# nanoporetech/dorado

Hardware: NVIDIA H100
Metric: basecalled samples/s (higher is better)
Workload: dtype f16 (fp32 accumulate; fp32 decode)

## Files before the change

dorado_b200/csrc/decode.cu:

```cuda
#include "decode.h"

#include "b200_crf_math.h"
#include "common.cuh"
#include "engine.h"
#include "nvtx.h"

#include <string>

namespace b200 {

namespace {

constexpr int kBeamW = 32;
constexpr uint32_t kCrcPoly = 0x82f63b78u;
constexpr uint32_t kCrcSeed = 0x12345678u;

template <int SL>
struct Dims {
    static constexpr int S = 1 << (2 * SL);
    static constexpr int C = 4 * S;
};

template <int SL>
struct ScanCfg {
    static constexpr int S = Dims<SL>::S, C = Dims<SL>::C, P4 = S / 4;
    static constexpr int SPT = S > 512 ? S / 512 : 1;
    static constexpr int NT = S / SPT;
    static constexpr int PITCH = P4 + 2;
};

__device__ __forceinline__ float clampf(float v, float c) {
    const float ce = c > 0.0f ? c : __int_as_float(0x7f800000);
    return fminf(fmaxf(v, -ce), ce);
}

template <int SL>
__global__ void __launch_bounds__(ScanCfg<SL>::S > 256 ? ScanCfg<SL>::S : 256)
        crf_bwd_scan_kernel(const __half* __restrict__ scores, float* __restrict__ bwd, int N, int T_pitch, float clamp_val,
                            float blank, const int32_t* __restrict__ lens, int stride) {
    using Cfg = ScanCfg<SL>;
    constexpr int S = Cfg::S, C = Cfg::C, P4 = Cfg::P4, PITCH = Cfg::PITCH;
    constexpr int CH = S >= 256 ? 1 : 256 / S;
    constexpr int PF = 4;
    const int g = threadIdx.x / S;
    const int v = threadIdx.x % S;
    const int chunk = blockIdx.x * CH + g;
    __shared__ __align__(16) float a[CH][2][S];
    __shared__ float st[CH][2][16 * PITCH];
    const bool active = chunk < N;
    const int chunk_c = active ? chunk : N - 1;
    const int T = lens ? min(T_pitch, __ldg(lens + chunk_c) / stride) : T_pitch;
    const uint2* srow = reinterpret_cast<const uint2*>(scores + (size_t)chunk_c * T_pitch * C) + v;
    constexpr int RS = C / 4;
    float* out = bwd + (size_t)chunk_c * (T_pitch + 1) * S;
    const int q = v % P4, top = v / P4;
    const int st_row = 4 * (v & 3), st_col = v >> 2;

    uint2 pf[PF];
#pragma unroll
    for (int k = 0; k < PF; ++k) {
        const int tt = T - 1 - k;
        if (tt >= 0) pf[k] = __ldg(srow + (size_t)tt * RS);
    }
    auto stage = [&](int buf, const uint2& r) {
        const __half2 h0 = *reinterpret_cast<const __half2*>(&r.x), h1 = *reinterpret_cast<const __half2*>(&r.y);
        const float2 f0 = __half22float2(h0), f1 = __half22float2(h1);
        float* d = &st[g][buf][st_row * PITCH + st_col];
        d[0] = clampf(f0.x, clamp_val);
        d[PITCH] = clampf(f0.y, clamp_val);
        d[2 * PITCH] = clampf(f1.x, clamp_val);
        d[3 * PITCH] = clampf(f1.y, clamp_val);
    };
    float own = 0.0f;
    a[g][0][v] = 0.0f;
    if (active) out[(size_t)T * S + v] = 0.0f;
    stage(0, pf[0]);
    if (T - 1 - PF >= 0) pf[0] = __ldg(srow + (size_t)(T - 1 - PF) * RS);
    if constexpr (S <= 32) __syncwarp(); else named_bar_sync(1 + g, S);

    int cur = 0;
    for (int t = T - 1; t >= 0; t -= PF) {
#pragma unroll
        for (int k = 0; k < PF; ++k) {
            const int tt = t - k;
            if (tt >= 0) {
                if (tt - 1 >= 0) {
                    stage(cur ^ 1, pf[(k + 1) % PF]);
                    if (tt - 1 - PF >= 0) pf[(k + 1) % PF] = __ldg(srow + (size_t)(tt - 1 - PF) * RS);
// ... 453 lines not shown
                    if (d) d[9] = clock64();
                    float vsum[SPT];
                    float lmax = B200_FLT_LOWEST;
#pragma unroll
                    for (int e = 0; e < SPT; ++e) {
                        const uint2 r = pf[k][e];
                        const float bw = pb[k][e];
                        if (t + PF < T) {
                            pf[k][e] = __ldg(reinterpret_cast<const uint2*>(srow + (size_t)(t + PF) * C) + e);
                            pb[k][e] = __ldg(brow + (size_t)(t + PF + 1) * S + e);
                        }
                        const float2 f0 = __half22float2(*reinterpret_cast<const __half2*>(&r.x));
                        const float2 f1 = __half22float2(*reinterpret_cast<const __half2*>(&r.y));
                        const float s0 = clampf(f0.x, clamp_val), s1 = clampf(f0.y, clamp_val);
                        const float s2 = clampf(f1.x, clamp_val), s3 = clampf(f1.y, clamp_val);
                        const int st = SPT * v + e;
                        {
                            const __half2 c0 = __floats2half2_rn(s0, s1), c1 = __floats2half2_rn(s2, s3);
                            uint2 pk;
                            pk.x = *reinterpret_cast<const uint32_t*>(&c0);
                            pk.y = *reinterpret_cast<const uint32_t*>(&c1);
                            *reinterpret_cast<uint2*>(&sc_row[g][slot][4 * st]) = pk;
                        }
                        bw_row[g][slot][st] = bw;
                        const int p = st >> 2;
                        f[e] = b200_lse5(B200_ADD(f[e], blank), B200_ADD(fa[g][cur][p], s0), B200_ADD(fa[g][cur][p + P4], s1),
                                         B200_ADD(fa[g][cur][p + 2 * P4], s2), B200_ADD(fa[g][cur][p + 3 * P4], s3));
                        fa[g][cur ^ 1][st] = f[e];
                        vsum[e] = B200_ADD(f[e], bw);
                        lmax = b200_fmaxf(lmax, vsum[e]);
                    }
                    float mx = warp_max(lmax);
                    if constexpr (NW > 1) {
                        if (lane == 0) red[g][0][wv] = mx;
                        named_bar_sync(BAR_SCAN, NT);
                        mx = red[g][0][0];
#pragma unroll
                        for (int w = 1; w < NW; ++w) mx = b200_fmaxf(mx, red[g][0][w]);
                    }
                    float ex[SPT];
                    float part = 0.0f;
#pragma unroll
                    for (int e = 0; e < SPT; ++e) {
                        ex[e] = b200_expf_nonpos(B200_SUB(vsum[e], mx));
                        part = e == 0 ? ex[0] : B200_ADD(part, ex[e]);
                    }
#pragma unroll
                    for (int o = 16; o >= 1; o >>= 1) part = B200_ADD(part, __shfl_xor_sync(0xffffffffu, part, o));
                    float z = part;
                    if constexpr (NW > 1) {
                        if (lane == 0) red[g][1][wv] = part;
                        named_bar_sync(BAR_SCAN, NT);
                        z = red[g][1][0];
#pragma unroll
                        for (int w = 1; w < NW; ++w) z = B200_ADD(z, red[g][1][w]);
                    }
#pragma unroll
                    for (int e = 0; e < SPT; ++e) post_row[g][slot][SPT * v + e] = B200_DIV(ex[e], z);
                    named_bar_arrive(BAR_FULL + slot, GT);
                    if (d) d[10] = clock64();
                    cur ^= 1;
                }
            }
        }
    } else {
        named_bar_sync(BAR_SCAN, GT);
        BeamLane me{0u, 0u, 0.0f};
        int width = beam_init<SL>(bw_row[g][1], bsm[g], me, W, lane);
        named_bar_sync(BAR_SCAN, GT);
        for (int t = 0; t < T; ++t) {
            const int slot = t & 1;
            long long* d = (dbg && chunk == 0 && t >= 100 && t < 108) ? dbg + (t - 100) * 16 : nullptr;
            if (d && lane == 0) d[7] = clock64();
            named_bar_sync(BAR_FULL + slot, GT);
            width = beam_step<SL>(sc_row[g][slot], bw_row[g][slot], post_row[g][slot], bsm[g], me, width, W, log_beam_cut, blank,
                                  t == T - 1, meta_out + (size_t)t * kBeamW, prob_out + (size_t)t * kBeamW, lane, d);
            if (t + 2 < T) named_bar_arrive(BAR_EMPTY + slot, GT);
        }
    }
}

constexpr int kWarpDecodeMaxChunks = 16;
constexpr int kWarpStPitch = 16 + 2;

struct WarpDecodeSmem {
    __align__(16) float fa[2][64];
    float st[16 * kWarpStPitch];
    __align__(16) __half sc_row[256];
    __align__(16) float bw_row[64];
    __align__(16) float post_row[64];
    BeamSmem bs;
};

__device__ __forceinline__ float4 clamped_scores(const uint2& r, float clamp_val) {
    const float2 f0 = __half22float2(*reinterpret_cast<const __half2*>(&r.x));
    const float2 f1 = __half22float2(*reinterpret_cast<const __half2*>(&r.y));
    return make_float4(clampf(f0.x, clamp_val), clampf(f0.y, clamp_val), clampf(f1.x, clamp_val), clampf(f1.y, clamp_val));
}

__global__ void __launch_bounds__(kWarpDecodeMaxChunks * 32, 1) crf_decode_warp_kernel(const __half* __restrict__ scores,
                                                                                      float* __restrict__ bwd,
                                                                                      uint2* __restrict__ beam,
                                                                                      int N,
                                                                                      int T_pitch,
                                                                                      float clamp_val,
                                                                                      float blank,
                                                                                      int W,
                                                                                      float log_beam_cut,
                                                                                      const int32_t* __restrict__ lens,
                                                                                      int stride) {
    constexpr int S = Dims<3>::S, C = Dims<3>::C, P4 = S / 4, PITCH = kWarpStPitch;
    constexpr int RS = C / 4;
    constexpr int PF = 4;
    extern __shared__ __align__(16) unsigned char warp_decode_smem[];
    const int w = threadIdx.x >> 5, lane = threadIdx.x & 31;
    const int chunk = blockIdx.x * (blockDim.x >> 5) + w;
    if (chunk >= N) return;
    WarpDecodeSmem& sm = reinterpret_cast<WarpDecodeSmem*>(warp_decode_smem)[w];
    const int T = lens ? min(T_pitch, __ldg(lens + chunk) / stride) : T_pitch;
    const uint2* srow = reinterpret_cast<const uint2*>(scores + (size_t)chunk * T_pitch * C);
    float* brow = bwd + (size_t)chunk * (T_pitch + 1) * S;
    const int s0 = lane, s1 = lane + 32;

    {
        const int q = lane & 15, top = lane >> 4;
        auto stage = [&](const uint2& r, int v) {
            const float4 f = clamped_scores(r, clamp_val);
            float* d = &sm.st[4 * (v & 3) * PITCH + (v >> 2)];
            d[0] = f.x;
            d[PITCH] = f.y;
            d[2 * PITCH] = f.z;
            d[3 * PITCH] = f.w;
        };
        uint2 pf[PF][2];
#pragma unroll
        for (int k = 0; k < PF; ++k) {
            const int tt = T - 1 - k;
            if (tt >= 0) {
                pf[k][0] = __ldg(srow + (size_t)tt * RS + s0);
                pf[k][1] = __ldg(srow + (size_t)tt * RS + s1);
            }
        }
        float own0 = 0.0f, own1 = 0.0f;
        sm.fa[0][s0] = 0.0f;
        sm.fa[0][s1] = 0.0f;
        brow[(size_t)T * S + s0] = 0.0f;
        brow[(size_t)T * S + s1] = 0.0f;
        int cur = 0;
        for (int t = T - 1; t >= 0; t -= PF) {
#pragma unroll
            for (int k = 0; k < PF; ++k) {
                const int tt = t - k;
                if (tt >= 0) {
                    stage(pf[k][0], s0);
                    stage(pf[k][1], s1);
                    if (tt - PF >= 0) {
                        pf[k][0] = __ldg(srow + (size_t)(tt - PF) * RS + s0);
                        pf[k][1] = __ldg(srow + (size_t)(tt - PF) * RS + s1);
                    }
                    __syncwarp();
                    const float4 nx = *reinterpret_cast<const float4*>(&sm.fa[cur][4 * q]);
                    const float* sa = &sm.st[top * PITCH + q];
                    const float* sb = &sm.st[(top + 2) * PITCH + q];
                    own0 = b200_lse5(B200_ADD(own0, blank), B200_ADD(nx.x, sa[0]), B200_ADD(nx.y, sa[4 * PITCH]),
                                     B200_ADD(nx.z, sa[8 * PITCH]), B200_ADD(nx.w, sa[12 * PITCH]));
                    own1 = b200_lse5(B200_ADD(own1, blank), B200_ADD(nx.x, sb[0]), B200_ADD(nx.y, sb[4 * PITCH]),
                                     B200_ADD(nx.z, sb[8 * PITCH]), B200_ADD(nx.w, sb[12 * PITCH]));
                    sm.fa[cur ^ 1][s0] = own0;
                    sm.fa[cur ^ 1][s1] = own1;
                    brow[(size_t)tt * S + s0] = own0;
                    brow[(size_t)tt * S + s1] = own1;
                    __syncwarp();
                    cur ^= 1;
                }
            }
        }
    }
    __syncwarp();

    uint32_t* meta_out = reinterpret_cast<uint32_t*>(beam) + (size_t)chunk * T_pitch * kBeamW;
    float* prob_out = reinterpret_cast<float*>(beam) + ((size_t)N + chunk) * T_pitch * kBeamW;
    sm.fa[0][s0] = 0.0f;
    sm.fa[0][s1] = 0.0f;
    sm.bw_row[s0] = brow[s0];
    sm.bw_row[s1] = brow[s1];
    __syncwarp();
    BeamLane me{0u, 0u, 0.0f};
    int width = beam_init<3>(sm.bw_row, sm.bs, me, W, lane);
    uint2 r0n{}, r1n{};
    float b0n = 0.0f, b1n = 0.0f;
    if (T > 0) {
        r0n = __ldg(srow + s0);
        r1n = __ldg(srow + s1);
        b0n = brow[S + s0];
        b1n = brow[S + s1];
    }
    float f0 = 0.0f, f1 = 0.0f;
    int cur = 0;
    const int p0 = s0 >> 2, p1 = s1 >> 2;
    for (int t = 0; t < T; ++t) {
        const uint2 r0 = r0n, r1 = r1n;
        const float bw0 = b0n, bw1 = b1n;
        if (t + 1 < T) {
            r0n = __ldg(srow + (size_t)(t + 1) * RS + s0);
            r1n = __ldg(srow + (size_t)(t + 1) * RS + s1);
            b0n = brow[(size_t)(t + 2) * S + s0];
            b1n = brow[(size_t)(t + 2) * S + s1];
        }
        const float4 c0 = clamped_scores(r0, clamp_val), c1 = clamped_scores(r1, clamp_val);
        {
            const __half2 h00 = __floats2half2_rn(c0.x, c0.y), h01 = __floats2half2_rn(c0.z, c0.w);
            const __half2 h10 = __floats2half2_rn(c1.x, c1.y), h11 = __floats2half2_rn(c1.z, c1.w);
            *reinterpret_cast<uint2*>(&sm.sc_row[4 * s0]) =
                    make_uint2(*reinterpret_cast<const uint32_t*>(&h00), *reinterpret_cast<const uint32_t*>(&h01));
            *reinterpret_cast<uint2*>(&sm.sc_row[4 * s1]) =
                    make_uint2(*reinterpret_cast<const uint32_t*>(&h10), *reinterpret_cast<const uint32_t*>(&h11));
        }
        sm.bw_row[s0] = bw0;
        sm.bw_row[s1] = bw1;
        const float* fc = sm.fa[cur];
        f0 = b200_lse5(B200_ADD(f0, blank), B200_ADD(fc[p0], c0.x), B200_ADD(fc[p0 + P4], c0.y), B200_ADD(fc[p0 + 2 * P4], c0.z),
                       B200_ADD(fc[p0 + 3 * P4], c0.w));
        f1 = b200_lse5(B200_ADD(f1, blank), B200_ADD(fc[p1], c1.x), B200_ADD(fc[p1 + P4], c1.y), B200_ADD(fc[p1 + 2 * P4], c1.z),
                       B200_ADD(fc[p1 + 3 * P4], c1.w));
        sm.fa[cur ^ 1][s0] = f0;
        sm.fa[cur ^ 1][s1] = f1;
        const float v0 = B200_ADD(f0, bw0), v1 = B200_ADD(f1, bw1);
        const float mx = warp_max(b200_fmaxf(v0, v1));
        const float e0 = b200_expf_nonpos(B200_SUB(v0, mx)), e1 = b200_expf_nonpos(B200_SUB(v1, mx));
        float z0 = e0, z1 = e1;
#pragma unroll
        for (int o = 16; o >= 1; o >>= 1) {
            z0 = B200_ADD(z0, __shfl_xor_sync(0xffffffffu, z0, o));
            z1 = B200_ADD(z1, __shfl_xor_sync(0xffffffffu, z1, o));
        }
        const float z = B200_ADD(z0, z1);
        sm.post_row[s0] = B200_DIV(e0, z);
        sm.post_row[s1] = B200_DIV(e1, z);
        __syncwarp();
        width = beam_step<3>(sm.sc_row, sm.bw_row, sm.post_row, sm.bs, me, width, W, log_beam_cut, blank, t == T - 1,
                             meta_out + (size_t)t * kBeamW, prob_out + (size_t)t * kBeamW, lane, nullptr);
        cur ^= 1;
    }
}

int warp_decode_chunks_per_cta(int N, int runners) {
    const int R = runners > 1 ? runners : 1;
    const int per = (int)(((long long)N * R + kNumSMs - 1) / kNumSMs);
    return per < 1 ? 1 : (per > kWarpDecodeMaxChunks ? kWarpDecodeMaxChunks : per);
}

constexpr int kTbTile = 32;
constexpr int kTbWarps = 2;

__host__ __device__ constexpr size_t traceback_warp_bytes(int T) {
    return ((size_t)kTbTile * kBeamW * 4 + (size_t)((T + 3) & ~3) * (4 + 4 + 2) + 16 + 15) & ~(size_t)15;
}

__global__ void __launch_bounds__(kTbWarps * 32) crf_traceback_kernel(const uint32_t* __restrict__ beam_meta,
                                                                      const float* __restrict__ beam_prob,
                                                                      int N,
                                                                      int T_pitch,
                                                                      const int32_t* __restrict__ lens,
                                                                      int stride,
                                                                      const b200_qtable* __restrict__ qtable,
                                                                      uint8_t* __restrict__ moves_out,
                                                                      char* __restrict__ seq_out,
                                                                      char* __restrict__ qstr_out,
                                                                      int32_t* __restrict__ n_bases_out) {
    extern __shared__ __align__(16) unsigned char tb_smem[];
    __shared__ b200_qtable qt;
    for (int i = threadIdx.x; i < (int)(sizeof(b200_qtable) / 4); i += blockDim.x) {
        reinterpret_cast<uint32_t*>(&qt)[i] = reinterpret_cast<const uint32_t*>(qtable)[i];
    }
    __syncthreads();
    const int w = threadIdx.x >> 5, lane = threadIdx.x & 31;
    const int chunk = blockIdx.x * kTbWarps + w;
    if (chunk >= N) return;
    const int T = lens ? min(T_pitch, __ldg(lens + chunk) / stride) : T_pitch;
    const int Tp = (T_pitch + 3) & ~3;
    unsigned char* base = tb_smem + (size_t)w * traceback_warp_bytes(T_pitch);
    uint32_t* tile = reinterpret_cast<uint32_t*>(base);
    uint32_t* path = tile + kTbTile * kBeamW;
    float* pprob = reinterpret_cast<float*>(path + Tp);
    uint16_t* bstart = reinterpret_cast<uint16_t*>(pprob + Tp);

    const uint32_t* mrow = beam_meta + (size_t)chunk * T_pitch * kBeamW + lane;
    uint32_t nxt[kTbTile];
    auto load_tile = [&](int t_hi) {
        const int t_lo = t_hi - kTbTile;
#pragma unroll
        for (int r = 0; r < kTbTile; ++r) {
            const int t = t_lo + r;
            nxt[r] = t >= 0 ? __ldg(mrow + (size_t)t * kBeamW) : 0u;
        }
    };
    if (T > 0) load_tile(T);
    uint32_t ei = 0;
    for (int t_hi = T; t_hi > 0; t_hi -= kTbTile) {
#pragma unroll
        for (int r = 0; r < kTbTile; ++r) tile[r * kBeamW + lane] = nxt[r];
        __syncwarp();
        if (t_hi - kTbTile > 0) load_tile(t_hi - kTbTile);
        if (lane == 0) {
            const int t_lo = t_hi - kTbTile;
            const int r_lo = t_lo < 0 ? -t_lo : 0;
            for (int r = kTbTile - 1; r >= r_lo; --r) {
                const uint32_t e = tile[r * kBeamW + ei];
                path[t_lo + r] = (e & 0xffffu) | ((((e >> 24) & 1u) ^ 1u) << 16) | (ei << 24);
                ei = (e >> 16) & 0xffu;
            }
        }
        __syncwarp();
    }
    if (lane == 0 && T > 0) path[0] |= 1u << 16;
    __syncwarp();
    {
        const float* prow = beam_prob + (size_t)chunk * T_pitch * kBeamW;
        for (int t = lane; t < T; t += 32) {
            pprob[t] = b200_pow0p4f(__ldg(prow + (size_t)t * kBeamW + (path[t] >> 24)));
        }
    }
    __syncwarp();

    int nb = 0;
    for (int t0 = 0; t0 < T; t0 += 32) {
        const int t = t0 + lane;
        const bool m = t < T && ((path[t] >> 16) & 1u);
        const uint32_t bal = __ballot_sync(0xffffffffu, m);
        if (m) bstart[nb + __popc(bal & ((1u << lane) - 1u))] = (uint16_t)t;
        nb += __popc(bal);
    }
    if (lane == 0) bstart[nb] = (uint16_t)T;
    __syncwarp();

    uint8_t* mo = moves_out + (size_t)chunk * T_pitch;
    char* so = seq_out + (size_t)chunk * T_pitch;
    char* qo = qstr_out + (size_t)chunk * T_pitch;
    for (int t = lane; t < T_pitch; t += 32) mo[t] = t < T ? (uint8_t)((path[t] >> 16) & 1u) : 0;
    for (int p = lane; p < T_pitch; p += 32) {
        char sc = 0, qc = 0;
        if (p < nb) {
            const int b0 = bstart[p], b1 = bstart[p + 1];
            float bp = 0.0f, tp = 0.0f;
            int base = 0;
            for (int blk = b0; blk < b1; ++blk) {
                base = path[blk] & 3;
                const float prob = pprob[blk];
                const float wrong = B200_DIV(B200_SUB(1.0f, prob), 3.0f);
                bp = B200_ADD(bp, prob);
#pragma unroll
                for (int k = 0; k < 4; ++k) tp = B200_ADD(tp, k == base ? prob : wrong);
            }
            sc = "ACGT"[path[b0] & 3];
            qc = b200_qtable_lookup(&qt, bp, tp);
        }
        so[p] = sc;
        qo[p] = qc;
    }
    if (lane == 0) n_bases_out[chunk] = nb;
}

size_t traceback_smem_bytes(int T) { return kTbWarps * traceback_warp_bytes(T); }

void launch_traceback(const DecodeArgs& a, cudaStream_t stream, ProfileSink* prof) {
    const size_t smem = traceback_smem_bytes(a.T);
    if (smem > 48 * 1024) ensure_dynamic_smem(crf_traceback_kernel, 200 * 1024);
    const int grid = (a.N + kTbWarps - 1) / kTbWarps;
    NvtxRange r("decode");
    const uint32_t* meta = reinterpret_cast<const uint32_t*>(a.beam);
    const float* prob = reinterpret_cast<const float*>(a.beam) + (size_t)a.N * a.T * kBeamW;
    crf_traceback_kernel<<<grid, kTbWarps * 32, smem, stream>>>(meta, prob, a.N, a.T, a.lens, a.stride, a.qtable, a.moves,
                                                                a.sequence, a.qstring, a.n_bases);
    if (prof) prof->mark("crf_traceback", stream);
}

void launch_decode_warp(const DecodeArgs& a, cudaStream_t stream, ProfileSink* prof) {
    {
        const int cpc = warp_decode_chunks_per_cta(a.N, a.runners);
        const int grid = (a.N + cpc - 1) / cpc;
        const size_t smem = (size_t)cpc * sizeof(WarpDecodeSmem);
        ensure_dynamic_smem(crf_decode_warp_kernel, (int)(kWarpDecodeMaxChunks * sizeof(WarpDecodeSmem)));
        NvtxRange r("beam_search");
        crf_decode_warp_kernel<<<grid, cpc * 32, smem, stream>>>(a.scores, a.bwd, a.beam, a.N, a.T, a.clamp_val, a.blank,
                                                                 a.beam_width, a.log_beam_cut, a.lens, a.stride);
        if (prof) prof->mark("crf_fwd_beam", stream);
    }
    launch_traceback(a, stream, prof);
    B200_CUDA(cudaGetLastError());
}

template <int SL>
void launch_decode(const DecodeArgs& a, cudaStream_t stream, ProfileSink* prof) {
    {
        constexpr int S = Dims<SL>::S;
        constexpr int CH = S >= 256 ? 1 : 256 / S;
        const int grid = (a.N + CH - 1) / CH;
        NvtxRange r("back_guides");
        crf_bwd_scan_kernel<SL><<<grid, S * CH, 0, stream>>>(a.scores, a.bwd, a.N, a.T, a.clamp_val, a.blank, a.lens, a.stride);
        if (prof) prof->mark("crf_bwd_scan", stream);
    }
    {
        using F = FwdCfg<SL>;
        const int grid = (a.N + F::CH - 1) / F::CH;
        NvtxRange r("beam_search");
        crf_fwd_beam_kernel<SL><<<grid, F::THREADS, 0, stream>>>(a.scores, a.bwd, a.beam, a.N, a.T, a.clamp_val, a.blank,
                                                                   a.beam_width, a.log_beam_cut, a.lens, a.stride, a.dbg);
        if (prof) prof->mark("crf_fwd_beam", stream);
    }
    launch_traceback(a, stream, prof);
    B200_CUDA(cudaGetLastError());
}

}

size_t decode_max_blocks() {
    int T = 65535;
    while (traceback_smem_bytes(T) > 200 * 1024) T -= 64;
    return (size_t)T;
}

void carve_decode_scratch(Bump& b, int N, int T, int state_len, float** bwd, uint2** beam) {
    const size_t S = (size_t)1 << (2 * state_len);
    *bwd = b.take<float>((size_t)N * (T + 1) * S * sizeof(float));
    *beam = b.take<uint2>((size_t)N * T * kBeamW * sizeof(uint2));
}

int decode_launches(int state_len) { return state_len == 3 ? 2 : 3; }

void decode_scores(const DecodeArgs& a, cudaStream_t stream, ProfileSink* prof) {
    if (a.beam_width < 1 || a.beam_width > kBeamW) {
        throw std::invalid_argument("b200 decode: beam_width must be in [1, 32]");
    }
    if (a.T < 1 || a.T > 65535 || a.N < 1) {
        throw std::invalid_argument("b200 decode: need 1 <= T <= 65535 and N >= 1");
    }
    if (!a.qtable) throw std::invalid_argument("b200 decode: quality table missing");
    if (a.lens && a.stride < 1) throw std::invalid_argument("b200 decode: chunk lengths need the model stride");
    if (traceback_smem_bytes(a.T) > 200 * 1024) {
        throw std::invalid_argument("b200 decode: " + std::to_string(a.T) + " blocks per chunk exceed what the traceback kernel "
                                    "holds in shared memory (about 10 700); use a smaller chunk size");
    }
    switch (a.state_len) {
        case 3: launch_decode_warp(a, stream, prof); break;
        case 4: launch_decode<4>(a, stream, prof); break;
        case 5: launch_decode<5>(a, stream, prof); break;
        default: throw std::invalid_argument("b200 decode: state_len must be 3, 4 or 5");
    }
}

}
```

dorado_b200/csrc/decode.h:

```cpp
#pragma once

#include <cuda_fp16.h>
#include <cuda_runtime.h>
#include <stddef.h>
#include <stdint.h>
#include "b200_crf_math.h"

namespace b200 {

struct DecodeArgs {
    const __half* scores;
    int N;
    int T;
    int state_len;
    float clamp_val;
    int beam_width;
    float log_beam_cut;
    float blank;
    float q_shift;
    float q_scale;
    const b200_qtable* qtable;
    const int32_t* lens;
    int stride;
    int runners;
    long long* dbg;
    float* bwd;
    uint2* beam;
    uint8_t* moves;
    char* sequence;
    char* qstring;
    int32_t* n_bases;
};

size_t decode_max_blocks();
class Bump;
void carve_decode_scratch(Bump& b, int N, int T, int state_len, float** bwd, uint2** beam);
int decode_launches(int state_len);
struct ProfileSink;
void decode_scores(const DecodeArgs& args, cudaStream_t stream, ProfileSink* prof = nullptr);

}
```

dorado_b200/csrc/engine.cu:

```cuda
#include "engine.h"

#include "b200_crf_math.h"
#include "decode.h"
#include "nvtx.h"

#include <algorithm>
#include <cstdio>
#include <cstdlib>
#include <cmath>
#include <cstring>
#include <limits>
#include <set>
#include <utility>
#include <vector>

namespace b200 {

void ensure_dynamic_smem(const void* kernel, int bytes) {
    static std::mutex mu;
    static std::set<std::pair<int, const void*>> done;
    int dev = 0;
    B200_CUDA(cudaGetDevice(&dev));
    std::lock_guard<std::mutex> lock(mu);
    if (done.count({dev, kernel})) return;
// ... 469 lines not shown
        run_decode(num_chunks);
        B200_CUDA(cudaEventRecord(m_ev[2], s));
        B200_CUDA(cudaStreamSynchronize(s));
        m_plan->check_errors();
        float ms = 0;
        B200_CUDA(cudaEventElapsedTime(&ms, m_ev[0], m_ev[1]));
        fwd += ms;
        B200_CUDA(cudaEventElapsedTime(&ms, m_ev[1], m_ev[2]));
        dec += ms;
    }
    *total_ms = fwd + dec;
    if (forward_ms) *forward_ms = fwd;
    if (decode_ms) *decode_ms = dec;
}

void pipelined_steps(Runner** rs, int R, int num_chunks, int iters, float* total_ms) {
    if (R < 1 || !rs || iters < 1) throw std::invalid_argument("pipelined_steps: bad arguments");
    for (int r = 0; r < R; ++r) {
        if (!rs[r]) throw std::invalid_argument("pipelined_steps: null runner");
        if (&rs[r]->m_engine != &rs[0]->m_engine) throw std::invalid_argument("pipelined_steps: runners of different engines");
        if (num_chunks < 1 || num_chunks > rs[r]->m_N) throw std::invalid_argument("pipelined_steps: num_chunks out of range");
        for (int q = 0; q < r; ++q) {
            if (rs[q] == rs[r]) throw std::invalid_argument("pipelined_steps: the same runner twice");
        }
    }
    std::vector<Runner*> order(rs, rs + R);
    std::sort(order.begin(), order.end());
    std::vector<std::unique_lock<std::mutex>> locks;
    for (Runner* r : order) locks.emplace_back(r->m_mutex);
    Runner& r0 = *rs[0];
    B200_CUDA(cudaSetDevice(r0.m_engine.device()));
    B200_CUDA(cudaEventRecord(r0.m_ev[0], r0.m_stream));
    for (int r = 1; r < R; ++r) B200_CUDA(cudaStreamWaitEvent(rs[r]->m_stream, r0.m_ev[0], 0));
    for (int i = 0; i < iters; ++i) {
        Runner& ru = *rs[i % R];
        ru.run_forward(num_chunks);
        ru.run_decode(num_chunks);
    }
    for (int r = 1; r < R; ++r) {
        B200_CUDA(cudaEventRecord(rs[r]->m_ev[2], rs[r]->m_stream));
        B200_CUDA(cudaStreamWaitEvent(r0.m_stream, rs[r]->m_ev[2], 0));
    }
    B200_CUDA(cudaEventRecord(r0.m_ev[1], r0.m_stream));
    B200_CUDA(cudaStreamSynchronize(r0.m_stream));
    for (int r = 0; r < R; ++r) rs[r]->m_plan->check_errors();
    B200_CUDA(cudaEventElapsedTime(total_ms, r0.m_ev[0], r0.m_ev[1]));
}

void Runner::forward_scores_to_host(int num_chunks, uint16_t* scores_out) {
    if (num_chunks < 1 || num_chunks > m_N) throw std::invalid_argument("forward_scores: num_chunks out of range");
    std::lock_guard<std::mutex> lock(m_mutex);
    B200_CUDA(cudaSetDevice(m_engine.device()));
    cudaStream_t s = m_stream;
    stage_input(num_chunks);
    run_forward(num_chunks);
    B200_CUDA(cudaMemcpyAsync(scores_out, m_dev.scores, (size_t)num_chunks * m_T_out * m_C * sizeof(__half),
                              cudaMemcpyDeviceToHost, s));
    B200_CUDA(cudaStreamSynchronize(s));
    m_plan->check_errors();
}

void ProfileSink::begin(cudaStream_t s) { mark("begin", s); }

void ProfileSink::mark(const char* name, cudaStream_t s) {
    cudaEvent_t e;
    B200_CUDA(cudaEventCreate(&e));
    B200_CUDA(cudaEventRecord(e, s));
    events.push_back(e);
    names.emplace_back(name);
}

std::vector<std::pair<std::string, float>> ProfileSink::report() {
    std::vector<std::pair<std::string, float>> out;
    for (size_t i = 1; i < events.size(); ++i) {
        float ms = 0;
        B200_CUDA(cudaEventElapsedTime(&ms, events[i - 1], events[i]));
        out.emplace_back(names[i], ms);
    }
    return out;
}

ProfileSink::~ProfileSink() {
    for (auto e : events) cudaEventDestroy(e);
}

std::string Runner::profile(int num_chunks) {
    if (num_chunks < 1 || num_chunks > m_N) throw std::invalid_argument("profile: num_chunks out of range");
    std::lock_guard<std::mutex> lock(m_mutex);
    B200_CUDA(cudaSetDevice(m_engine.device()));
    cudaStream_t s = m_stream;
    ProfileSink sink;
    sink.begin(s);
    m_plan->run(s, &sink);
    m_engine.gpu_launches += m_plan->launches();
    run_decode(num_chunks, &sink);
    B200_CUDA(cudaStreamSynchronize(s));
    m_plan->check_errors();
    std::string out;
    for (auto& kv : sink.report()) out += kv.first + "=" + std::to_string(kv.second) + ";";
    return out;
}

void Runner::debug_read_workspace(uint64_t offset, uint64_t bytes, void* dst) {
    if (offset + bytes > m_dev.ws_bytes) throw std::invalid_argument("debug_read_workspace: out of range");
    std::lock_guard<std::mutex> lock(m_mutex);
    B200_CUDA(cudaSetDevice(m_engine.device()));
    B200_CUDA(cudaStreamSynchronize(m_stream));
    B200_CUDA(cudaMemcpy(dst, static_cast<unsigned char*>(m_dev.ws) + offset, bytes, cudaMemcpyDeviceToHost));
}

size_t runner_device_bytes(Engine& engine, int batch_size, int chunk_size) {
    Bump sizing;
    carve_runner(sizing, engine, batch_size, chunk_size);
    return sizing.used();
}

int benchmark_batch_sizes(Engine& engine, int chunk_size, int granularity, int max_batch_size, int32_t* batch_sizes,
                          float* ms_per_chunk, int capacity) {
    if (granularity < 1 || max_batch_size < granularity) throw std::invalid_argument("benchmark_batch_sizes: bad range");
    int count = 0;
    for (int bs = granularity; bs <= max_batch_size; bs += granularity, ++count) {
        float best = std::numeric_limits<float>::max();
        {
            Runner scratch(engine, bs, chunk_size);
            scratch.fill_synthetic_input();
            for (int i = 0; i < 2; ++i) {
                float total = 0, fwd = 0, dec = 0;
                scratch.step_device(bs, 1, &total, &fwd, &dec);
                best = std::min(best, total / (float)bs);
            }
        }
        if (count < capacity) {
            if (batch_sizes) batch_sizes[count] = bs;
            if (ms_per_chunk) ms_per_chunk[count] = best;
        }
    }
    return count;
}

int select_batch_size(const int32_t* batch_sizes, const float* ms_per_chunk, int count, int max_batch_size, int granularity,
                      float time_penalty) {
    if (!batch_sizes || !ms_per_chunk || count < 1) throw std::invalid_argument("select_batch_size: empty table");
    if (!(time_penalty >= 0.0f)) throw std::invalid_argument("select_batch_size: negative time penalty");
    std::vector<int> kept;
    float best = std::numeric_limits<float>::max();
    for (int i = 0; i < count; ++i) {
        if (i > 0 && batch_sizes[i] <= batch_sizes[i - 1]) throw std::invalid_argument("select_batch_size: batch sizes must ascend");
        if (ms_per_chunk[i] < best) {
            best = ms_per_chunk[i];
            kept.push_back(i);
        }
    }
    if (kept.empty()) throw std::invalid_argument("select_batch_size: no finite timing");
    const float threshold = best * (1.0f + time_penalty);
    size_t last = 0;
    while (last < kept.size() && !(ms_per_chunk[kept[last]] <= threshold)) ++last;
    int selected = granularity;
    for (size_t k = 0; k <= last && k < kept.size(); ++k) {
        if (batch_sizes[kept[k]] <= max_batch_size) selected = batch_sizes[kept[k]];
    }
    return selected;
}

void decode_host_scores(int device, const uint16_t* scores, int N, int T, int C, float clamp_val,
                        const b200_decoder_options& opts, uint8_t* moves, char* sequence, char* qstring,
                        int32_t* n_bases) {
// ... 88 lines not shown
```

dorado_b200/csrc/engine.h:

```cpp
#pragma once

#include "b200call.h"
#include "b200_crf_math.h"
#include "frontend.h"
#include "common.cuh"
#include "lstm_kernels.h"

#include <atomic>
#include <condition_variable>
#include <memory>
#include <mutex>
#include <stdexcept>
#include <string>
#include <vector>

namespace b200 {

struct Unsupported : std::runtime_error {
    using std::runtime_error::runtime_error;
};

class Bump {
public:
    Bump() = default;
// ... 76 lines not shown

class Engine {
public:
    Engine(const b200_model_desc& desc, const b200_tensor* tensors, int num_tensors, int device);
    ~Engine();
    const b200_model_desc& desc() const { return m_desc; }
    int device() const { return m_device; }
    cudaStream_t stream() const { return m_stream; }
    Model& model() { return *m_model; }
    std::mutex& stats_mutex() { return m_stats_mutex; }
    b200_stats stats() const;

    void terminate();
    void restart();
    bool terminated() const { return m_terminated.load(); }
    void set_low_latency(bool on) { m_low_latency.store(on); }
    void set_num_runners(int n) { m_model->num_runners_hint = n < 1 ? 1 : (n > 16 ? 16 : n); }
    int num_runners() const { return m_model->num_runners_hint; }
    bool low_latency() const { return m_low_latency.load(); }
    void batch_timeouts_ms(int* first_chunk_ms, int* last_chunk_ms) const;
    struct CallGuard {
        explicit CallGuard(Engine& e);
        ~CallGuard();
        Engine& eng;
    };

    std::atomic<int64_t> batches_called{0};
    std::atomic<int64_t> gpu_launches{0};
    std::atomic<int64_t> arena_bytes{0};
    double model_decode_ms = 0, h2d_ms = 0, d2h_ms = 0;

private:
    b200_model_desc m_desc;
    int m_device;
    cudaStream_t m_stream = nullptr;
    std::unique_ptr<Model> m_model;
    mutable std::mutex m_stats_mutex;
    std::atomic<bool> m_terminated{false};
    std::atomic<bool> m_low_latency{false};
    std::mutex m_life_mutex;
    std::condition_variable m_life_cv;
    int m_in_flight = 0;
};

class Runner;
void pipelined_steps(Runner** runners, int n_runners, int num_chunks, int iters, float* total_ms);

struct RunnerBuffers {
    b200_qtable* qtable = nullptr;
    int32_t* lens = nullptr;
    __half* input = nullptr;
    __half* scores = nullptr;
    void* ws = nullptr;
    size_t ws_bytes = 0;
    float* bwd = nullptr;
    uint2* beam = nullptr;
    unsigned char* out = nullptr;
    size_t out_bytes = 0;
};

class Runner {
public:
    friend void pipelined_steps(Runner** runners, int n_runners, int num_chunks, int iters, float* total_ms);
    Runner(Engine& engine, int batch_size, int chunk_size);
    ~Runner();
    int batch_size() const { return m_N; }
    int chunk_size() const { return m_T_in; }
    int out_len() const { return m_T_out; }
    uint16_t* input();
    void set_decoder_options(const b200_decoder_options& o);
    void accept_chunk_f16(int idx, const uint16_t* samples, int64_t len);
    void accept_chunk_f32(int idx, const float* samples, int64_t len);
    bool variable_chunk_sizes() const;
    void accept_chunk_var_f16(int idx, const uint16_t* samples, int64_t len);
    void accept_raw_chunk(int idx, const b200_raw_chunk& chunk);
    void debug_read_input(int num_chunks, uint16_t* input_out);
    b200_result call_chunks(int num_chunks);
    void upload();
    void fill_synthetic_input();
    void step_device(int num_chunks, int iters, float* total_ms, float* forward_ms, float* decode_ms);
    void forward_scores_to_host(int num_chunks, uint16_t* scores_out);
    void debug_read_workspace(uint64_t offset, uint64_t bytes, void* dst);
    std::string profile(int num_chunks);
    std::string plan_info() const { return m_plan ? m_plan->info() : std::string(); }

private:
    void init();
    void release();
    bool m_counted = false;
    void stage_input(int n);
    void clear_raw_slot(int idx);
    void run_forward(int n);
    void run_decode(int n, ProfileSink* prof = nullptr);

    Engine& m_engine;
    cudaStream_t m_stream = nullptr;
    std::mutex m_mutex;
    int m_N, m_T_in, m_T_out, m_C;
    b200_decoder_options m_opts;
    uint16_t* m_h_input = nullptr;
    unsigned char* m_h_out = nullptr;
    int16_t* m_h_raw = nullptr;
    RawSlot* m_h_slots = nullptr;
    int16_t* m_d_raw = nullptr;
    RawSlot* m_d_slots = nullptr;
    int m_num_raw = 0;
    Arena m_arena;
    RunnerBuffers m_dev;
    std::unique_ptr<ForwardPlan> m_plan;
    void upload_qtable();
    int32_t* m_h_lens = nullptr;
    int32_t* m_h_nmoves = nullptr;
    cudaEvent_t m_ev[4] = {nullptr, nullptr, nullptr, nullptr};
};

class ModBaseEngine {
public:
    ModBaseEngine(const b200_modbase_desc& desc, const b200_tensor* tensors, int num_tensors, int device);
    ~ModBaseEngine();
    ModBaseEngine(const ModBaseEngine&) = delete;
    ModBaseEngine& operator=(const ModBaseEngine&) = delete;
    const b200_modbase_desc& desc() const { return m_desc; }
    int device() const { return m_device; }

    int sig_len = 0;
    int seq_len = 0;
    int t_enc = 0;
    int T = 0;
    int out_len = 0;
    float* sig12_w = nullptr;
    __half* sig3_w = nullptr;
    float* sig3_b = nullptr;
    float* seq1_w = nullptr;
    __half* seq2_w = nullptr;
    float* seq2_b = nullptr;
    __half* merge_w = nullptr;
    float* merge_b = nullptr;
    LstmLayerWeights lstm[2];
    float* fc_w = nullptr;
    float* fc_b = nullptr;
    float* up_w = nullptr;
    float* up_b = nullptr;

private:
    b200_modbase_desc m_desc;
    int m_device;
};

struct ModBasePlan;
class ModBaseRunner {
public:
    ModBaseRunner(ModBaseEngine& engine, int batch_size);
    ~ModBaseRunner();
    int batch_size() const { return m_N; }
    const ModBaseEngine& engine() const { return m_engine; }
    void accept_chunk(int idx, const uint16_t* signal, int64_t sig_len, const int8_t* kmers, int64_t kmer_elems);
    const uint16_t* call_chunks(int num_chunks);
    std::string profile();
    void debug_read_workspace(uint64_t offset, uint64_t bytes, void* dst);

private:
    void init();
    void release();
    void run(ProfileSink* prof);

    ModBaseEngine& m_engine;
    int m_N;
// ... 93 lines not shown
```

Baseline: 1.111 billion.

## Split warp decode into forward-scan and beam-search warps with mbarrier ring

Each chunk in the warp decode kernel now gets two warps. One runs the backward and forward CRF scans and writes per-step scores, backward values and posteriors into a four-slot shared-memory ring. The other consumes the ring with beam_step, and the two are synchronised by full/empty mbarriers. The aim is to overlap forward-scan latency with the serial beam search. In exchange the block size doubles, shared memory per chunk grows, and mbarrier wait overhead is added. A plan_info helper reporting the decode CTA count is also added.

Measured after the change: 1.132 billion (median of 6 runs). +1.9%, better.

```diff
diff --git a/dorado_b200/csrc/decode.cu b/dorado_b200/csrc/decode.cu
--- a/dorado_b200/csrc/decode.cu
+++ b/dorado_b200/csrc/decode.cu
@@ -4,6 +4,7 @@
 #include "common.cuh"
 #include "engine.h"
 #include "nvtx.h"
+#include "tc.cuh"
 
 #include <string>
 
@@ -623,14 +624,23 @@
 
 constexpr int kWarpDecodeMaxChunks = 16;
 constexpr int kWarpStPitch = 16 + 2;
+constexpr int kDecodeRing = 4;
+
+struct DecodeSlot {
+    __align__(16) __half sc_row[256];
+    __align__(16) float bw_row[64];
+    __align__(16) float post_row[64];
+};
 
 struct WarpDecodeSmem {
     __align__(16) float fa[2][64];
     float st[16 * kWarpStPitch];
-    __align__(16) __half sc_row[256];
-    __align__(16) float bw_row[64];
-    __align__(16) float post_row[64];
+    __align__(16) float bw0[64];
+    DecodeSlot ring[kDecodeRing];
     BeamSmem bs;
+    uint64_t full[kDecodeRing];
+    uint64_t empty[kDecodeRing];
+    uint64_t init;
 };
 
 __device__ __forceinline__ float4 clamped_scores(const uint2& r, float clamp_val) {
@@ -639,7 +649,7 @@
     return make_float4(clampf(f0.x, clamp_val), clampf(f0.y, clamp_val), clampf(f1.x, clamp_val), clampf(f1.y, clamp_val));
 }
 
-__global__ void __launch_bounds__(kWarpDecodeMaxChunks * 32, 1) crf_decode_warp_kernel(const __half* __restrict__ scores,
+__global__ void __launch_bounds__(kWarpDecodeMaxChunks * 64, 1) crf_decode_warp_kernel(const __half* __restrict__ scores,
                                                                                       float* __restrict__ bwd,
                                                                                       uint2* __restrict__ beam,
                                                                                       int N,
@@ -654,11 +664,42 @@
     constexpr int RS = C / 4;
     constexpr int PF = 4;
     extern __shared__ __align__(16) unsigned char warp_decode_smem[];
+    const int cpc = blockDim.x >> 6;
     const int w = threadIdx.x >> 5, lane = threadIdx.x & 31;
-    const int chunk = blockIdx.x * (blockDim.x >> 5) + w;
+    const bool scan_warp = w < cpc;
+    const int c = scan_warp ? w : w - cpc;
+    const int chunk = blockIdx.x * cpc + c;
+    WarpDecodeSmem& sm = reinterpret_cast<WarpDecodeSmem*>(warp_decode_smem)[c];
+    if (scan_warp && lane == 0) {
+#pragma unroll
+        for (int k = 0; k < kDecodeRing; ++k) {
+            tc::mbar_init(&sm.full[k], 32);
+            tc::mbar_init(&sm.empty[k], 32);
+        }
+        tc::mbar_init(&sm.init, 32);
+        tc::fence_barrier_init();
+    }
+    __syncthreads();
     if (chunk >= N) return;
-    WarpDecodeSmem& sm = reinterpret_cast<WarpDecodeSmem*>(warp_decode_smem)[w];
     const int T = lens ? min(T_pitch, __ldg(lens + chunk) / stride) : T_pitch;
+
+    if (!scan_warp) {
+        uint32_t* meta_out = reinterpret_cast<uint32_t*>(beam) + (size_t)chunk * T_pitch * kBeamW;
+        float* prob_out = reinterpret_cast<float*>(beam) + ((size_t)N + chunk) * T_pitch * kBeamW;
+        tc::mbar_wait_silent(&sm.init, 0);
+        BeamLane me{0u, 0u, 0.0f};
+        int width = beam_init<3>(sm.bw0, sm.bs, me, W, lane);
+        for (int t = 0; t < T; ++t) {
+            const int slot = t % kDecodeRing;
+            tc::mbar_wait_silent(&sm.full[slot], (uint32_t)(t / kDecodeRing) & 1u);
+            const DecodeSlot& d = sm.ring[slot];
+            width = beam_step<3>(d.sc_row, d.bw_row, d.post_row, sm.bs, me, width, W, log_beam_cut, blank, t == T - 1,
+                                 meta_out + (size_t)t * kBeamW, prob_out + (size_t)t * kBeamW, lane, nullptr);
+            tc::mbar_arrive(&sm.empty[slot]);
+        }
+        return;
+    }
+
     const uint2* srow = reinterpret_cast<const uint2*>(scores + (size_t)chunk * T_pitch * C);
     float* brow = bwd + (size_t)chunk * (T_pitch + 1) * S;
     const int s0 = lane, s1 = lane + 32;
@@ -716,18 +757,15 @@
                 }
             }
         }
+        sm.bw0[s0] = own0;
+        sm.bw0[s1] = own1;
+        tc::mbar_arrive(&sm.init);
     }
     __syncwarp();
 
-    uint32_t* meta_out = reinterpret_cast<uint32_t*>(beam) + (size_t)chunk * T_pitch * kBeamW;
-    float* prob_out = reinterpret_cast<float*>(beam) + ((size_t)N + chunk) * T_pitch * kBeamW;
     sm.fa[0][s0] = 0.0f;
     sm.fa[0][s1] = 0.0f;
-    sm.bw_row[s0] = brow[s0];
-    sm.bw_row[s1] = brow[s1];
     __syncwarp();
-    BeamLane me{0u, 0u, 0.0f};
-    int width = beam_init<3>(sm.bw_row, sm.bs, me, W, lane);
     uint2 r0n{}, r1n{};
     float b0n = 0.0f, b1n = 0.0f;
     if (T > 0) {
@@ -749,16 +787,6 @@
             b1n = brow[(size_t)(t + 2) * S + s1];
         }
         const float4 c0 = clamped_scores(r0, clamp_val), c1 = clamped_scores(r1, clamp_val);
-        {
-            const __half2 h00 = __floats2half2_rn(c0.x, c0.y), h01 = __floats2half2_rn(c0.z, c0.w);
-            const __half2 h10 = __floats2half2_rn(c1.x, c1.y), h11 = __floats2half2_rn(c1.z, c1.w);
-            *reinterpret_cast<uint2*>(&sm.sc_row[4 * s0]) =
-                    make_uint2(*reinterpret_cast<const uint32_t*>(&h00), *reinterpret_cast<const uint32_t*>(&h01));
-            *reinterpret_cast<uint2*>(&sm.sc_row[4 * s1]) =
-                    make_uint2(*reinterpret_cast<const uint32_t*>(&h10), *reinterpret_cast<const uint32_t*>(&h11));
-        }
-        sm.bw_row[s0] = bw0;
-        sm.bw_row[s1] = bw1;
         const float* fc = sm.fa[cur];
         f0 = b200_lse5(B200_ADD(f0, blank), B200_ADD(fc[p0], c0.x), B200_ADD(fc[p0 + P4], c0.y), B200_ADD(fc[p0 + 2 * P4], c0.z),
                        B200_ADD(fc[p0 + 3 * P4], c0.w));
@@ -776,11 +804,23 @@
             z1 = B200_ADD(z1, __shfl_xor_sync(0xffffffffu, z1, o));
         }
         const float z = B200_ADD(z0, z1);
-        sm.post_row[s0] = B200_DIV(e0, z);
-        sm.post_row[s1] = B200_DIV(e1, z);
+        const int slot = t % kDecodeRing;
+        if (t >= kDecodeRing) tc::mbar_wait_silent(&sm.empty[slot], (uint32_t)(t / kDecodeRing - 1) & 1u);
+        DecodeSlot& d = sm.ring[slot];
+        {
+            const __half2 h00 = __floats2half2_rn(c0.x, c0.y), h01 = __floats2half2_rn(c0.z, c0.w);
+            const __half2 h10 = __floats2half2_rn(c1.x, c1.y), h11 = __floats2half2_rn(c1.z, c1.w);
+            *reinterpret_cast<uint2*>(&d.sc_row[4 * s0]) =
+                    make_uint2(*reinterpret_cast<const uint32_t*>(&h00), *reinterpret_cast<const uint32_t*>(&h01));
+            *reinterpret_cast<uint2*>(&d.sc_row[4 * s1]) =
+                    make_uint2(*reinterpret_cast<const uint32_t*>(&h10), *reinterpret_cast<const uint32_t*>(&h11));
+        }
+        d.bw_row[s0] = bw0;
+        d.bw_row[s1] = bw1;
+        d.post_row[s0] = B200_DIV(e0, z);
+        d.post_row[s1] = B200_DIV(e1, z);
+        tc::mbar_arrive(&sm.full[slot]);
         __syncwarp();
-        width = beam_step<3>(sm.sc_row, sm.bw_row, sm.post_row, sm.bs, me, width, W, log_beam_cut, blank, t == T - 1,
-                             meta_out + (size_t)t * kBeamW, prob_out + (size_t)t * kBeamW, lane, nullptr);
         cur ^= 1;
     }
 }
@@ -923,7 +963,7 @@
         const size_t smem = (size_t)cpc * sizeof(WarpDecodeSmem);
         ensure_dynamic_smem(crf_decode_warp_kernel, (int)(kWarpDecodeMaxChunks * sizeof(WarpDecodeSmem)));
         NvtxRange r("beam_search");
-        crf_decode_warp_kernel<<<grid, cpc * 32, smem, stream>>>(a.scores, a.bwd, a.beam, a.N, a.T, a.clamp_val, a.blank,
+        crf_decode_warp_kernel<<<grid, cpc * 64, smem, stream>>>(a.scores, a.bwd, a.beam, a.N, a.T, a.clamp_val, a.blank,
                                                                  a.beam_width, a.log_beam_cut, a.lens, a.stride);
         if (prof) prof->mark("crf_fwd_beam", stream);
     }
@@ -967,6 +1007,12 @@
     *beam = b.take<uint2>((size_t)N * T * kBeamW * sizeof(uint2));
 }
 
+std::string decode_plan_info(int N, int state_len, int runners) {
+    if (state_len != 3 || N < 1) return std::string();
+    const int cpc = warp_decode_chunks_per_cta(N, runners);
+    return "crf_fwd_beam.ctas=" + std::to_string((N + cpc - 1) / cpc);
+}
+
 int decode_launches(int state_len) { return state_len == 3 ? 2 : 3; }
 
 void decode_scores(const DecodeArgs& a, cudaStream_t stream, ProfileSink* prof) {
diff --git a/dorado_b200/csrc/decode.h b/dorado_b200/csrc/decode.h
--- a/dorado_b200/csrc/decode.h
+++ b/dorado_b200/csrc/decode.h
@@ -4,6 +4,7 @@
 #include <cuda_runtime.h>
 #include <stddef.h>
 #include <stdint.h>
+#include <string>
 #include "b200_crf_math.h"
 
 namespace b200 {
@@ -36,6 +37,7 @@
 class Bump;
 void carve_decode_scratch(Bump& b, int N, int T, int state_len, float** bwd, uint2** beam);
 int decode_launches(int state_len);
+std::string decode_plan_info(int N, int state_len, int runners);
 struct ProfileSink;
 void decode_scores(const DecodeArgs& args, cudaStream_t stream, ProfileSink* prof = nullptr);
 
diff --git a/dorado_b200/csrc/engine.cu b/dorado_b200/csrc/engine.cu
--- a/dorado_b200/csrc/engine.cu
+++ b/dorado_b200/csrc/engine.cu
@@ -575,6 +575,13 @@
 
 ProfileSink::~ProfileSink() {
     for (auto e : events) cudaEventDestroy(e);
+}
+
+std::string Runner::plan_info() const {
+    std::string s = m_plan ? m_plan->info() : std::string();
+    const std::string d = decode_plan_info(m_N, m_engine.desc().state_len, m_engine.num_runners());
+    if (!d.empty()) s += (s.empty() ? "" : ";") + d;
+    return s;
 }
 
 std::string Runner::profile(int num_chunks) {
diff --git a/dorado_b200/csrc/engine.h b/dorado_b200/csrc/engine.h
--- a/dorado_b200/csrc/engine.h
+++ b/dorado_b200/csrc/engine.h
@@ -182,7 +182,7 @@
     void forward_scores_to_host(int num_chunks, uint16_t* scores_out);
     void debug_read_workspace(uint64_t offset, uint64_t bytes, void* dst);
     std::string profile(int num_chunks);
-    std::string plan_info() const { return m_plan ? m_plan->info() : std::string(); }
+    std::string plan_info() const;
 
 private:
     void init();
```
